# Litianyu141/Gen-FVGN-steady

Measured on AMD Instinct MI355X. Metric: training iters/sec, 50k-cell cylinder mesh (fwd + loss + bwd + Adam, batch resident in HBM), higher is better.
Workload: dtype f32

## Files before the change

### gen-fvgn-steady_amd/csrc/cfwd.hip

```cpp
#include <cstdlib>

#include "tchain_kernel.h"

#include "gfv_limits.h"
int* gfv_internal_status_ptr();

namespace {

constexpr float CF_SH = 16.0f;
constexpr float CF_SH_INV = 1.0f / 16.0f;
constexpr float CF_SH_LIMIT = 2048.0f;

__device__ __forceinline__ void cf_barrier() {
  asm volatile("s_waitcnt lgkmcnt(0)\n\ts_barrier" ::: "memory");
}

template <int KT0, int TG, int NW>
struct CfLds {
  static constexpr int KTB = KT0 > 4 ? KT0 : 4;
  static constexpr int B0 = 0;
  static constexpr int B1 = TG * KTB * 2048;
  static constexpr int SINV = B1 + TG * 8192;
  static constexpr int LNP = SINV + TG * 64;
  static constexpr int TOTAL = LNP + TG * 16 * NW * 8;
};

template <int KT0, int N0, int TG, bool PADD, int LOWP, bool RAGIN, int NW = 4, bool FINLN = true>
__global__ __launch_bounds__(64 * NW, NW == 8 ? 4 : 2) void cfwd_kernel(const gfv_rowtile_args_t A, int* status) {
  static_assert(TG == 2 || TG == 4, "one loader wave per group");
  static_assert(NW == 4 || NW == 8, "32 or 16 columns per wave");
  constexpr int NT = 8 / NW;
  using LY = CfLds<KT0, TG, NW>;
  constexpr bool BF = LOWP == 2;
  __shared__ __attribute__((aligned(16))) char lds[LY::TOTAL];
  char* b0 = lds + LY::B0;
  char* b1 = lds + LY::B1;
  float* sinv = reinterpret_cast<float*>(lds + LY::SINV);
  float* lnp = reinterpret_cast<float*>(lds + LY::LNP);

  const int w = __builtin_amdgcn_readfirstlane(threadIdx.x >> 6);
  const int lane = threadIdx.x & 63, j = lane & 15, g = lane >> 4;
  const int tile = PADD ? gfv_xcd_tile(blockIdx.x, gridDim.x) : (int)blockIdx.x;
  const int row0 = tile * (16 * TG);
  if (row0 >= A.M) return;
  const int ngt = min(TG, (A.M - row0 + 15) >> 4);
  const int c0 = 16 * NT * w + 4 * g;
  const float invw = 1.0f / gfv_pow2_scale(*A.wmax);

  gfv_f16x8 wh[NT][KT0 > 4 ? KT0 : 4], wl[NT][KT0 > 4 ? KT0 : 4];
  {
    const gfv_f16x8* im = reinterpret_cast<const gfv_f16x8*>(A.layer[0].Wh) + (size_t)(NT * w) * 128 + lane;
#pragma unroll
    for (int T = 0; T < KT0; ++T)
#pragma unroll
      for (int n = 0; n < NT; ++n) {
        wh[n][T] = im[T * 1024 + n * 128];
        if (!LOWP) wl[n][T] = im[T * 1024 + n * 128 + 64];
      }
  }
  float4 ps[PADD ? TG : 1][NT], pr[PADD ? TG : 1][NT];
  if (PADD) {
#pragma unroll
    for (int q = 0; q < TG; ++q) {
      const int row = min(row0 + 16 * q + j, A.M - 1);
      const float* s = A.padd + (size_t)A.padd_s[row] * A.padd_ld + c0;
      const float* r = A.padd + (size_t)A.padd_r[row] * A.padd_ld + 128 + c0;
#pragma unroll
      for (int n = 0; n < NT; ++n) { ps[q][n] = ld4(s + 16 * n); pr[q][n] = ld4(r + 16 * n); }
    }
  }
  if (w < TG) {
    const int row = min(row0 + 16 * w + j, A.M - 1);
    float v[2 * KT0][4];
    if (RAGIN) {
      const int width = A.seg[0].width;
      const float* rp = A.seg[0].ptr + (size_t)row * A.seg[0].ld;
#pragma unroll
      for (int u = 0; u < 2; ++u)
#pragma unroll
        for (int e = 0; e < 4; ++e) {
          const int col = 16 * u + 4 * g + e;
          v[u][e] = col < width ? rp[col] : 0.f;
        }
    } else {
      const float* p0 = A.seg[0].ptr + (size_t)row * A.seg[0].ld + 4 * g;
      const float* p1 = p0;
      if (N0 < 2 * KT0) p1 = A.seg[1].ptr + (size_t)row * A.seg[1].ld + 4 * g;
#pragma unroll
      for (int u = 0; u < 2 * KT0; ++u) {
        const float4 t = ld4(u < N0 ? p0 + 16 * u : p1 + 16 * (u - N0));
        v[u][0] = t.x; v[u][1] = t.y; v[u][2] = t.z; v[u][3] = t.w;
      }
    }
    float m0 = 0.f, m1 = 0.f;
#pragma unroll
    for (int u = 0; u < 2 * KT0; ++u) {
      m0 = max3_abs(m0, v[u][0], v[u][1]);
      m1 = max3_abs(m1, v[u][2], v[u][3]);
    }
    const float s = gfv_pow2_scale(row_max4(max3_abs(0.f, m0, m1)));
    if (g == 0) sinv[w * 16 + j] = 1.0f / s;
    gfv_uint4* dst = reinterpret_cast<gfv_uint4*>(b0 + (size_t)w * KT0 * 2048) + lane;
#pragma unroll
    for (int T = 0; T < KT0; ++T) {
      float e[8];
#pragma unroll
      for (int r = 0; r < 4; ++r) { e[r] = v[2 * T][r] * s; e[4 + r] = v[2 * T + 1][r] * s; }
      gfv_uint4 hi, lo;
      gfv_split8_t<BF>(e, hi, lo);
      dst[(2 * T) * 64] = hi;
      if (!LOWP) dst[(2 * T + 1) * 64] = lo;
    }
  }
  float4 bias[3][NT];
#pragma unroll
  for (int l = 0; l < 3; ++l) {
    const float* bp = (FINLN || l < 2) ? A.layer[l].bias : nullptr;
#pragma unroll
    for (int n = 0; n < NT; ++n) bias[l][n] = bp ? ld4(bp + c0 + 16 * n) : make_float4(0.f, 0.f, 0.f, 0.f);
  }
  float mabs = 0.f;
  cf_barrier();

  floatx4 acc[TG][NT];
  auto mma = [&](const char* xbuf, auto ktc) {
    constexpr int KT = decltype(ktc)::value;
#pragma unroll
    for (int q = 0; q < TG; ++q)
#pragma unroll
      for (int n = 0; n < NT; ++n) acc[q][n] = floatx4{0.f, 0.f, 0.f, 0.f};
#pragma unroll
    for (int T = 0; T < KT; ++T) {
#pragma unroll
      for (int q = 0; q < TG; ++q) {
        const gfv_f16x8* f = reinterpret_cast<const gfv_f16x8*>(xbuf + (size_t)(q * KT + T) * 2048) + lane;
        const gfv_f16x8 xh = f[0];
        if (!LOWP) {
          const gfv_f16x8 xl = f[64];
#pragma unroll
          for (int n = 0; n < NT; ++n) {
            acc[q][n] = __builtin_amdgcn_mfma_f32_16x16x32_f16(wl[n][T], xh, acc[q][n], 0, 0, 0);
            acc[q][n] = __builtin_amdgcn_mfma_f32_16x16x32_f16(wh[n][T], xl, acc[q][n], 0, 0, 0);
          }
        }
#pragma unroll
        for (int n = 0; n < NT; ++n) acc[q][n] = gfv_mma_hh<BF>(wh[n][T], xh, acc[q][n]);
      }
    }
  };
  auto load_w = [&](const void* image) {
    const gfv_f16x8* im = reinterpret_cast<const gfv_f16x8*>(image) + (size_t)(NT * w) * 128 + lane;
#pragma unroll
    for (int T = 0; T < 4; ++T)
#pragma unroll
      for (int n = 0; n < NT; ++n) {
        wh[n][T] = im[T * 1024 + n * 128];
        if (!LOWP) wl[n][T] = im[T * 1024 + n * 128 + 64];
      }
  };
  auto hidden = [&](int layer, char* xout, float* save) {
#pragma unroll
    for (int q = 0; q < TG; ++q) {
      const int row = row0 + 16 * q + j;
      const bool live = q < ngt && row < A.M;
      const float si = layer == 0 ? sinv[q * 16 + j] : CF_SH_INV;
      float a[4 * NT];
#pragma unroll
      for (int n = 0; n < NT; ++n) {
        const float4 b = bias[layer][n];
        float v[4] = {(acc[q][n][0] * si) * invw + b.x, (acc[q][n][1] * si) * invw + b.y, (acc[q][n][2] * si) * invw + b.z,
                      (acc[q][n][3] * si) * invw + b.w};
        if (PADD && layer == 0) {
          v[0] += ps[PADD ? q : 0][n].x + pr[PADD ? q : 0][n].x; v[1] += ps[PADD ? q : 0][n].y + pr[PADD ? q : 0][n].y;
          v[2] += ps[PADD ? q : 0][n].z + pr[PADD ? q : 0][n].z; v[3] += ps[PADD ? q : 0][n].w + pr[PADD ? q : 0][n].w;
        }
        if (save && live) st4(save + (size_t)row * 128 + c0 + 16 * n, v);
        const gfv_f2 g01 = gfv_gelu2(gfv_f2{v[0], v[1]}), g23 = gfv_gelu2(gfv_f2{v[2], v[3]});
        a[4 * n + 0] = g01.x; a[4 * n + 1] = g01.y; a[4 * n + 2] = g23.x; a[4 * n + 3] = g23.y;
      }
      float m = 0.f;
#pragma unroll
      for (int e = 0; e < 4 * NT; e += 2) m = max3_abs(m, a[e], a[e + 1]);
      mabs = fmaxf(mabs, live ? m : 0.f);
      if constexpr (NT == 2) {
        float e8[8];
#pragma unroll
        for (int e = 0; e < 8; ++e) e8[e] = a[e] * CF_SH;
        gfv_uint4 hi, lo;
        gfv_split8_t<BF>(e8, hi, lo);
        gfv_uint4* dst = reinterpret_cast<gfv_uint4*>(xout + (size_t)(q * 4 + w) * 2048) + lane;
        dst[0] = hi;
        if (!LOWP) dst[64] = lo;
      } else {
        unsigned h0, h1, l0, l1;
        gfv_split_pair_t<BF>(a[0] * CF_SH, a[1] * CF_SH, h0, l0);
        gfv_split_pair_t<BF>(a[2] * CF_SH, a[3] * CF_SH, h1, l1);
        char* dst = xout + (size_t)(q * 4 + (w >> 1)) * 2048 + lane * 16 + (w & 1) * 8;
        *reinterpret_cast<uint2*>(dst) = make_uint2(h0, h1);
        if (!LOWP) *reinterpret_cast<uint2*>(dst + 1024) = make_uint2(l0, l1);
      }
    }
  };

  mma(b0, std::integral_constant<int, KT0>{});
  load_w(A.layer[1].Wh);
  hidden(0, b1, A.layer[0].save);
  cf_barrier();
  mma(b1, std::integral_constant<int, 4>{});
  load_w(A.layer[2].Wh);
  hidden(1, b0, A.layer[1].save);
  float4 gam[NT], bet[NT];
  if constexpr (FINLN) {
#pragma unroll
    for (int n = 0; n < NT; ++n) { gam[n] = ld4(A.fin_gamma + c0 + 16 * n); bet[n] = ld4(A.fin_beta + c0 + 16 * n); }
  }
  float4 rres[TG][NT];
  if (A.res[0]) {
#pragma unroll
    for (int q = 0; q < TG; ++q) {
      const float* rp = A.res[0] + (size_t)min(row0 + 16 * q + j, A.M - 1) * A.res_ld[0] + c0;
#pragma unroll
      for (int n = 0; n < NT; ++n) rres[q][n] = ld4(rp + 16 * n);
    }
  }
  cf_barrier();
  if constexpr (!FINLN) {
    if (w == 0) {
      mma(b0, std::integral_constant<int, 4>{});
      const int ncol = A.layer[2].N;
      const float* bp = A.layer[2].bias;
#pragma unroll
      for (int q = 0; q < TG; ++q) {
        const int row = row0 + 16 * q + j;
        if (q < ngt && row < A.M) {
#pragma unroll
          for (int r = 0; r < 4; ++r) {
            const int col = 4 * g + r;
            if (col < ncol) A.out[0][(size_t)row * A.out_ld[0] + col] = (acc[q][0][r] * CF_SH_INV) * invw + (bp ? bp[col] : 0.f);
          }
        }
      }
    }
    if (mabs > CF_SH_LIMIT) atomicOr(status, 2);
    return;
  }
  mma(b0, std::integral_constant<int, 4>{});
  const int hcols = (A.hidden > 0 && A.hidden < 128) ? A.hidden : 128;
  float y[TG][4 * NT];
#pragma unroll
  for (int q = 0; q < TG; ++q) {
    const int row = row0 + 16 * q + j;
    const bool live = q < ngt && row < A.M;
    float s = 0.f;
#pragma unroll
    for (int n = 0; n < NT; ++n) {
      const float4 b = bias[2][n];
      float v[4] = {(acc[q][n][0] * CF_SH_INV) * invw + b.x, (acc[q][n][1] * CF_SH_INV) * invw + b.y,
                    (acc[q][n][2] * CF_SH_INV) * invw + b.z, (acc[q][n][3] * CF_SH_INV) * invw + b.w};
      if (A.fin_presave && live) st4(A.fin_presave + (size_t)row * 128 + c0 + 16 * n, v);
#pragma unroll
      for (int r = 0; r < 4; ++r) {
        y[q][4 * n + r] = v[r];
        s += v[r];
      }
    }
    const float mw = row_sum(s) * (1.0f / (16.0f * NT));
    float m2 = 0.f;
#pragma unroll
    for (int e = 0; e < 4 * NT; ++e) {
      const float d = y[q][e] - mw;
      m2 += d * d;
    }
    m2 = row_sum(m2);
    if (g == 0) *reinterpret_cast<float2*>(lnp + ((q * 16 + j) * NW + w) * 2) = make_float2(mw, m2);
  }
  cf_barrier();
  {
    const float inv_h = 1.0f / (float)hcols, npad = (float)(128 - hcols);
#pragma unroll
    for (int q = 0; q < TG; ++q) {
      const int row = row0 + 16 * q + j;
      const bool live = q < ngt && row < A.M;
      const float4* pp = reinterpret_cast<const float4*>(lnp + (q * 16 + j) * 2 * NW);
      float m128, m2a;
      if constexpr (NW == 4) {
        const float4 p0 = pp[0], p1 = pp[1];
        m128 = ((p0.x + p0.z) + (p1.x + p1.z)) * 0.25f;
        const float e0 = p0.x - m128, e1 = p0.z - m128, e2 = p1.x - m128, e3 = p1.z - m128;
        m2a = ((p0.y + p0.w) + (p1.y + p1.w)) + 32.0f * ((e0 * e0 + e1 * e1) + (e2 * e2 + e3 * e3));
      } else {
        const float4 p0 = pp[0], p1 = pp[1], p2 = pp[2], p3 = pp[3];
        m128 = (((p0.x + p0.z) + (p1.x + p1.z)) + ((p2.x + p2.z) + (p3.x + p3.z))) * 0.125f;
        const float e0 = p0.x - m128, e1 = p0.z - m128, e2 = p1.x - m128, e3 = p1.z - m128, e4 = p2.x - m128, e5 = p2.z - m128,
                    e6 = p3.x - m128, e7 = p3.z - m128;
        m2a = (((p0.y + p0.w) + (p1.y + p1.w)) + ((p2.y + p2.w) + (p3.y + p3.w))) +
              16.0f * (((e0 * e0 + e1 * e1) + (e2 * e2 + e3 * e3)) + ((e4 * e4 + e5 * e5) + (e6 * e6 + e7 * e7)));
      }
      const float mean = hcols == 128 ? m128 : (m128 * 128.0f) * inv_h;
      const float dm = m128 - mean;
      const float m2 = hcols == 128 ? m2a : (m2a + 128.0f * dm * dm) - npad * (mean * mean);
      const float rstd = rsqrtf(m2 * inv_h + 1e-5f);
      if (A.fin_stats && live && w == 0 && g == 0) *reinterpret_cast<float2*>(A.fin_stats + 2 * (size_t)row) = make_float2(mean, rstd);
#pragma unroll
      for (int n = 0; n < NT; ++n) {
        const float4 ga = gam[n], be = bet[n];
        float o[4] = {(y[q][4 * n + 0] - mean) * rstd * ga.x + be.x, (y[q][4 * n + 1] - mean) * rstd * ga.y + be.y,
                      (y[q][4 * n + 2] - mean) * rstd * ga.z + be.z, (y[q][4 * n + 3] - mean) * rstd * ga.w + be.w};
        if (live) {
          if (A.out_nores) st4(A.out_nores + (size_t)row * 128 + c0 + 16 * n, o);
          if (A.res[0]) { o[0] += rres[q][n].x; o[1] += rres[q][n].y; o[2] += rres[q][n].z; o[3] += rres[q][n].w; }
          st4(A.out[0] + (size_t)row * A.out_ld[0] + c0 + 16 * n, o);
        }
      }
    }
  }
  if (mabs > CF_SH_LIMIT) atomicOr(status, 2);
}

inline bool cf_al16(const void* p) { return (reinterpret_cast<size_t>(p) & 15) == 0; }

template <int KT0, int N0, bool PADD, bool RAGIN, bool FINLN = true>
void cf_launch(const gfv_rowtile_args_t& a, int lowp, hipStream_t stream) {
  int* st = gfv_internal_status_ptr();
  constexpr int tg = 2;
  const int tiles = (a.M + 16 * tg - 1) / (16 * tg);
  const dim3 grid(PADD ? gfv_xcd_grid(tiles) : tiles), blk(512);
  if (lowp == 2) GFV_LAUNCH((cfwd_kernel<KT0, N0, 2, PADD, 2, RAGIN, 8, FINLN>), grid, blk, 0, stream, a, st);
  else if (lowp) GFV_LAUNCH((cfwd_kernel<KT0, N0, 2, PADD, 1, RAGIN, 8, FINLN>), grid, blk, 0, stream, a, st);
  else GFV_LAUNCH((cfwd_kernel<KT0, N0, 2, PADD, 0, RAGIN, 8, FINLN>), grid, blk, 0, stream, a, st);
}

}

int gfv_internal_cfwd_try(const gfv_rowtile_args_t* a, int lowp, hipStream_t stream, int dry) {
  if (!gfv_internal_status_ptr()) return 0;
  const int on = gfv_internal_limit(GFV_LIM_CFWD_ON);
  const int max_m = gfv_internal_limit(GFV_LIM_CFWD_MAX_M);
  if (!on || a->nlayers != 3 || a->M > max_m || a->M < 1 || (a->flags & (GFV_CHAIN_ROW_OWNER | GFV_CHAIN_COLUMN_OWNER))) return 0;
  const bool dec = a->fin_op == GFV_FIN_PLAIN && a->layer[2].N >= 1 && a->layer[2].N <= 16 && !a->res[0] && !a->out_nores && !a->fin_presave &&
                   !a->fin_stats && !a->padd && a->nseg == 1 && a->layer[0].K == 128;
  if (a->in_op != GFV_IN_NONE || !a->wmax) return 0;
  if (!dec && (a->fin_op != GFV_FIN_LN || !a->fin_gamma || !a->fin_beta)) return 0;
  if (a->in_add || a->gadd || a->in_save || a->in_aux || a->ln_partial || a->gscale || a->dw_partial || a->in_stats || a->fin_aux) return 0;
  for (int l = 0; l < 3; ++l) {
    const gfv_layer_t& L = a->layer[l];
    if (!L.Wh || (L.N != 128 && !(dec && l == 2)) || L.aux || L.bias2 || (L.bias && !cf_al16(L.bias) && !(dec && l == 2))) return 0;
    if (L.op != (l < 2 ? GFV_OP_BIAS_GELU : GFV_OP_NONE)) return 0;
    if (l > 0 && L.K != 128) return 0;
    if (L.save && !cf_al16(L.save)) return 0;
  }
  if (a->layer[2].save) return 0;
  if (!a->out[0] || a->out[1] || a->out[2] || (!dec && ((a->out_ld[0] & 3) || !cf_al16(a->out[0]))) || a->res[1] || a->res[2]) return 0;
  if (a->res[0] && ((a->res_ld[0] & 3) || !cf_al16(a->res[0]))) return 0;
  if ((a->out_nores && !cf_al16(a->out_nores)) || (a->fin_presave && !cf_al16(a->fin_presave)) ||
      (!dec && (!cf_al16(a->fin_gamma) || !cf_al16(a->fin_beta))))
    return 0;
  if (a->fin_stats && (reinterpret_cast<size_t>(a->fin_stats) & 7)) return 0;
  for (int i = 0; i < a->nseg; ++i)
    if (a->seg[i].idx || a->seg[i].csr_rowptr || a->seg[i].csr_scale || a->seg[i].save) return 0;
  const int K0 = a->layer[0].K;
  int shape = -1;
  auto plain = [&](int i, int width) {
    const gfv_seg_t& s = a->seg[i];
    return s.width == width && (s.ld & 3) == 0 && cf_al16(s.ptr);
  };
  if (a->padd) {
    if (a->nseg == 1 && K0 == 128 && plain(0, 128) && a->padd_s && a->padd_r && a->padd_ld >= 256 && (a->padd_ld & 3) == 0 && cf_al16(a->padd))
      shape = 1;
  } else if (a->nseg == 2 && K0 == 192 && plain(0, 64) && plain(1, 128)) {
    shape = 0;
  } else if (dec) {
    if (plain(0, 128)) shape = 4;
  } else if (a->nseg == 1 && K0 == 128 && plain(0, 128)) {
    shape = 2;
  } else if (a->nseg == 1 && K0 <= 32 && a->seg[0].width == K0) {
    shape = 3;
  }
  if (shape < 0) return 0;
  if (dry) return 1;
  if (shape == 0) cf_launch<6, 4, false, false>(*a, lowp, stream);
  else if (shape == 1) cf_launch<4, 8, true, false>(*a, lowp, stream);
  else if (shape == 2) cf_launch<4, 8, false, false>(*a, lowp, stream);
  else if (shape == 4) cf_launch<4, 8, false, false, false>(*a, lowp, stream);
  else cf_launch<1, 2, false, true>(*a, lowp, stream);
  return 1;
}
```

### gen-fvgn-steady_amd/csrc/gfv_limits.h

```cpp
#pragma once
enum {
  GFV_LIM_CBWD_ON = 0,
  GFV_LIM_CBWD_MAX_M,
  GFV_LIM_CFWD_ON,
  GFV_LIM_CFWD_MAX_M,
  GFV_LIM_CTRANS_ON,
  GFV_LIM_CTRANS_MAX_M,
  GFV_LIM_LIN1S_ON,
  GFV_LIM_LIN1S_MAX_M,
  GFV_LIM_COUNT
};
int gfv_internal_limit(int which);
```

### gen-fvgn-steady_amd/csrc/rowtile.hip

```cpp
#include <atomic>
#include <stdio.h>
#include <stdlib.h>
#include <mutex>
#include "gfv_common.h"
#include "gfv_limits.h"
#include "gfv_prof.h"
#include "../../include/gfv.h"

namespace {
constexpr int BM = 64;
}

int gfv_internal_tchain_launch(const gfv_rowtile_args_t* args, int ragged, int f16, hipStream_t stream);

static std::atomic<int> g_f16_default{-1};
static thread_local int g_f16split = -1;
static int f16_default() {
  int d = g_f16_default.load(std::memory_order_relaxed);
  if (d < 0) {
    const char* e = getenv("GFV_F16SPLIT");
    d = e ? ((atoi(e) == 2 || atoi(e) == 3) ? atoi(e) : (atoi(e) != 0)) : 1;
    int expect = -1;
    if (!g_f16_default.compare_exchange_strong(expect, d)) d = expect;
  }
  return d;
}
extern "C" int gfv_f16split_enabled(void) { return g_f16split >= 0 ? g_f16split : f16_default(); }
extern "C" int gfv_set_f16split(int32_t on) {
  g_f16_default.store((on == 2 || on == 3) ? on : (on ? 1 : 0));
  g_f16split = -1;
  return GFV_OK;
}
extern "C" int gfv_set_f16split_thread(int32_t on) {
  if (on < -1 || on > 3) return GFV_ERR_ARG;
  g_f16split = on;
  return GFV_OK;
}
static int f16_mode() { return gfv_f16split_enabled(); }

static thread_local int g_hidden = 128;
extern "C" int gfv_hidden_size(void) { return g_hidden; }
extern "C" int gfv_set_hidden_size(int32_t h) {
  if (h < 16 || h > 128 || (h & 15)) return GFV_ERR_ARG;
  g_hidden = h;
  return GFV_OK;
}

static thread_local int g_last_path = -1;
extern "C" int gfv_rowtile_last_path(void) { return g_last_path; }
namespace {
struct LimitDef { const char* env; int dflt; };
const LimitDef k_limits[GFV_LIM_COUNT] = {
    {"GFV_CBWD", 1},        {"GFV_CBWD_MAX_M", 25000},      {"GFV_CFWD", 1},          {"GFV_CFWD_MAX_M", 250000},
    {"GFV_CTRANS", 1},         {"GFV_CTRANS_MAX_M", 16384},
    {"GFV_LIN1S", 1},       {"GFV_LIN1S_MAX_M", 16384}};
int g_limit[GFV_LIM_COUNT];
bool g_limit_set[GFV_LIM_COUNT];
std::once_flag g_limit_once;
void limits_init() {
  for (int i = 0; i < GFV_LIM_COUNT; ++i) {
    const char* e = getenv(k_limits[i].env);
    g_limit[i] = e ? atoi(e) : k_limits[i].dflt;
    g_limit_set[i] = false;
  }
}
}
int gfv_internal_limit(int which) {
  std::call_once(g_limit_once, limits_init);
  return (which >= 0 && which < GFV_LIM_COUNT) ? g_limit[which] : 0;
}
extern "C" int gfv_get_limit(int32_t which) { return (which >= 0 && which < GFV_LIM_COUNT) ? gfv_internal_limit(which) : -1; }
extern "C" int gfv_set_limit(int32_t which, int32_t value) {
  if (which < 0 || which >= GFV_LIM_COUNT) return GFV_ERR_ARG;
  std::call_once(g_limit_once, limits_init);
  if (value < 0) {
    const char* e = getenv(k_limits[which].env);
    g_limit[which] = e ? atoi(e) : k_limits[which].dflt;
  } else {
    g_limit[which] = value;
  }
  return GFV_OK;
}
extern "C" const char* gfv_limit_name(int32_t which) { return (which >= 0 && which < GFV_LIM_COUNT) ? k_limits[which].env : nullptr; }

static thread_local int g_last_ln_rows = 0;
extern "C" int gfv_rowtile_last_ln_rows(void) { return g_last_ln_rows; }

extern "C" int gfv_rowtile_tiles(int32_t M) { return (M + BM - 1) / BM; }

static int rowtile_chain_impl(const gfv_rowtile_args_t* args, void* stream);
extern "C" int gfv_rowtile_chain(const gfv_rowtile_args_t* args, void* stream) {
  if (!args) return GFV_ERR_ARG;
  if (args->product_form < 0 || args->product_form > 4 || (args->hidden != 0 && (args->hidden < 16 || args->hidden > 128 || (args->hidden & 15))))
    return GFV_ERR_ARG;
  if (args->product_form == 0 && args->hidden == 0) return rowtile_chain_impl(args, stream);
  const int f0 = g_f16split, h0 = g_hidden;
  if (args->product_form) g_f16split = args->product_form - 1;
  if (args->hidden) g_hidden = args->hidden;
  const int rc = rowtile_chain_impl(args, stream);
  g_f16split = f0;
  g_hidden = h0;
  return rc;
}
int gfv_internal_lin1_try(const gfv_rowtile_args_t* a, int lowp, hipStream_t stream, int dry);
int gfv_internal_cfwd_try(const gfv_rowtile_args_t* a, int lowp, hipStream_t stream, int dry);
bool gfv_internal_wimg_form_ok(const float* wmax);
int gfv_internal_cbwd_try(const gfv_rowtile_args_t* a, int lowp, hipStream_t stream, int dry);
static int cfwd_try(const gfv_rowtile_args_t* args, int lowp, hipStream_t stream, int dry) {
  if (args->nlayers != 3 || (args->fin_op != GFV_FIN_LN && args->fin_op != GFV_FIN_PLAIN)) return 0;
  gfv_rowtile_args_t local = *args;
  local.hidden = g_hidden;
  return gfv_internal_cfwd_try(&local, lowp, stream, dry);
}
static int cbwd_try(const gfv_rowtile_args_t* args, int lowp, hipStream_t stream, int dry) {
  if (args->in_op != GFV_IN_LNBWD || args->dw_partial || !args->in_stats) return 0;
  gfv_rowtile_args_t local = *args;
  local.hidden = g_hidden;
  return gfv_internal_cbwd_try(&local, lowp, stream, dry);
}
static int rowtile_chain_impl(const gfv_rowtile_args_t* args, void* stream) {
  if (!args || args->M < 0 || args->nlayers < 1 || args->nlayers > 3 || args->nseg < 1 || args->nseg > 3) return GFV_ERR_ARG;
  if (args->M == 0) {
    g_last_ln_rows = 0;
    return GFV_OK;
  }
  for (int i = 0; i < args->nseg; ++i)
    if (args->seg[i].width < 1 || args->seg[i].width > 128) return GFV_ERR_ARG;
  for (int l = 0; l + 1 < args->nlayers; ++l)
    if (args->layer[l].N != 128 || args->layer[l + 1].K != 128) return GFV_ERR_ARG;
  int k0 = 0;
  for (int i = 0; i < args->nseg; ++i) k0 += args->seg[i].width;
  if (k0 != args->layer[0].K) return GFV_ERR_ARG;
  const gfv_layer_t& last = args->layer[args->nlayers - 1];
  if (last.N > 384 || last.N < 1) return GFV_ERR_ARG;
  if ((args->rc_Wh[0] || args->rc_Wh[1]) && !args->dw_partial) return GFV_ERR_ARG;
  if (args->padd && (args->nlayers < 2 || args->padd_ld < 256 || (args->padd_ld & 3) || !args->padd_s || !args->padd_r)) return GFV_ERR_ARG;
  for (int l = 0; l < args->nlayers; ++l)
    if (args->layer[l].ldw != 0 && args->layer[l].ldw < args->layer[l].K) return GFV_ERR_ARG;
  if (last.N > 128 && (last.N & 15)) return GFV_ERR_ARG;
  if ((args->fin_op != GFV_FIN_PLAIN || args->in_op == GFV_IN_LN || args->in_op == GFV_IN_LNBWD) &&
      (args->fin_op != GFV_FIN_PLAIN ? last.N != 128 : false))
    return GFV_ERR_ARG;
  if ((args->in_op == GFV_IN_LN || args->in_op == GFV_IN_LNBWD) && (args->nseg != 1 || args->seg[0].width != 128))
    return GFV_ERR_ARG;
  bool fast_t = true;
  for (int i = 0; i < args->nseg; ++i) fast_t = fast_t && (args->seg[i].width % 32 == 0) && (args->seg[i].ld % 4 == 0);
  for (int l = 0; l < args->nlayers; ++l) {
    const bool lastl = (l == args->nlayers - 1);
    fast_t = fast_t && (args->layer[l].K % 4 == 0) && (args->layer[l].ldw % 4 == 0) && (args->layer[l].N % (lastl ? 64 : 128) == 0);
  }
  if (args->fin_op != GFV_FIN_PLAIN) fast_t = fast_t && last.N == 128;
  for (int c = 0; c < 3; ++c) {
    if (args->out[c]) fast_t = fast_t && (args->out_ld[c] % 4 == 0);
    if (args->res[c]) fast_t = fast_t && (args->res_ld[c] % 4 == 0);
  }
  bool rag_t = !fast_t && args->in_op != GFV_IN_LNBWD && args->fin_op != GFV_FIN_LNBWD;
  for (int l = 0; l + 1 < args->nlayers; ++l) rag_t = rag_t && args->layer[l].N == 128;
  if (last.N > 128) rag_t = rag_t && (last.N % 64 == 0);
  if (last.N % 16) rag_t = rag_t && last.op != GFV_OP_MUL_DGELU && args->fin_op == GFV_FIN_PLAIN && !args->out_nores;
  if (args->in_op == GFV_IN_LN) rag_t = rag_t && args->seg[0].width == 128 && (args->seg[0].ld % 4 == 0);
  if (args->gadd) rag_t = rag_t && args->seg[0].width == 128 && (args->seg[0].ld % 4 == 0);
  for (int l = 1; l < args->nlayers; ++l) rag_t = rag_t && (args->layer[l].K == 128);
  {
    bool csr = false;
    for (int i = 0; i < args->nseg; ++i) {
      const gfv_seg_t& sg = args->seg[i];
      csr = csr || sg.csr_rowptr != nullptr || sg.save != nullptr;
      if (sg.csr_rowptr && (!sg.idx || (i == 0 && args->in_add))) return GFV_ERR_ARG;
    }
    if (csr && (!fast_t || args->in_op == GFV_IN_LNBWD || args->fin_op == GFV_FIN_LNBWD))
      return GFV_ERR_ARG;
  }
  bool f16 = (fast_t || rag_t) && f16_mode() != 0 && args->wmax != nullptr;
  for (int l = 0; l < args->nlayers; ++l) f16 = f16 && args->layer[l].Wh != nullptr;
  for (int i = 0; i + 1 < args->nseg; ++i) f16 = f16 && (args->seg[i].width % 32 == 0);
  if (f16 && !gfv_internal_wimg_form_ok(args->wmax)) return GFV_ERR_ARG;
  for (int l = 0; l < args->nlayers; ++l)
    if ((!args->layer[l].W || args->layer[l].bias2) && !f16) return GFV_ERR_ARG;
  if (!fast_t && !rag_t) {
    static const bool dbg = getenv("GFV_ROWTILE_DEBUG") != nullptr;
    if (dbg)
      fprintf(stderr, "[gfv] gfv_rowtile_chain: unsupported shape M=%d nseg=%d widths=%d,%d,%d ld0=%d nlayers=%d K0=%d Nlast=%d out_ld=%d in_op=%d fin_op=%d\n",
              args->M, args->nseg, args->seg[0].width, args->nseg > 1 ? args->seg[1].width : 0,
              args->nseg > 2 ? args->seg[2].width : 0, args->seg[0].ld, args->nlayers, args->layer[0].K, last.N,
              args->out_ld[0], args->in_op, args->fin_op);
    return GFV_ERR_ARG;
  }
  void* tok = nullptr;
  if (gfv_prof_enabled()) {
    double fl = 0, by = 0;
    for (int l = 0; l < args->nlayers; ++l) {
      fl += 2.0 * args->M * (double)args->layer[l].K * args->layer[l].N;
      by += 4.0 * ((double)args->layer[l].K * args->layer[l].N + args->layer[l].N);
      if (args->layer[l].save) by += 4.0 * args->M * args->layer[l].N;
      if (args->layer[l].aux) by += 4.0 * args->M * args->layer[l].N;
    }
    by += 4.0 * args->M * (double)args->layer[0].K + 4.0 * args->M * (double)last.N;
    for (int i = 0; i < args->nseg; ++i) if (args->seg[i].idx) by += 4.0 * args->M;
    if (args->in_aux || args->fin_aux) by += 4.0 * args->M * 128.0;
    if (args->in_save) by += 4.0 * args->M * 128.0;
    if (args->fin_presave) by += 4.0 * args->M * 128.0;
    if (args->out_nores) by += 4.0 * args->M * 128.0;
    if (args->padd) by += 4.0 * args->M * 258.0;
    for (int c = 0; c < 3; ++c) if (args->res[c]) by += 4.0 * args->M * 128.0;
    const int lnm = args->in_op == GFV_IN_LNBWD ? 1 : (args->fin_op == GFV_FIN_LNBWD ? 2 : 0);
    int kind = fast_t ? GFV_K_TCHAIN0 + lnm : GFV_K_TCHAIN_RAG;
    for (int i = 0; i < args->nseg; ++i)
      if (args->seg[i].csr_rowptr || args->seg[i].save) kind = GFV_K_TCHAIN_CSR;
    if (fast_t && f16 && args->nlayers == 1 && gfv_internal_lin1_try(args, f16_mode() >= 2 ? f16_mode() - 1 : 0, (hipStream_t)stream, 1))
      kind = GFV_K_LIN1;
    if (f16 && cfwd_try(args, f16_mode() >= 2 ? f16_mode() - 1 : 0, (hipStream_t)stream, 1))
      kind = GFV_K_COLCHAIN_FWD;
    if (args->dw_partial) {
      kind = GFV_K_COLCHAIN_BWD;
      const int nfused = 2 + (args->rc_Wh[0] ? 2 : 0);
      fl += nfused * 2.0 * args->M * 128.0 * 128.0;
      by += 8.0 * args->M + 4.0 * (double)gfv_rowtile_dw_partials_m(args->M) * (double)args->dw_partial_stride;
    }
    tok = gfv_prof_begin(kind, fl, by, (hipStream_t)stream);
  }
  g_last_path = (fast_t ? 1 : 2) + (f16 ? 4 : 0);
  g_last_ln_rows = (args->M + BM - 1) / BM;
  if (args->dw_partial && !(fast_t && f16)) return GFV_ERR_ARG;
  if (fast_t && f16 && args->nlayers == 1 && gfv_internal_lin1_try(args, f16_mode() >= 2 ? f16_mode() - 1 : 0, (hipStream_t)stream, 0)) {
    g_last_path += 32;
  } else if (f16 && !args->dw_partial && cfwd_try(args, f16_mode() >= 2 ? f16_mode() - 1 : 0, (hipStream_t)stream, 0)) {
    g_last_path += 64;
  } else if (fast_t && f16 && cbwd_try(args, f16_mode() >= 2 ? f16_mode() - 1 : 0, (hipStream_t)stream, 0)) {
    g_last_path += 128;
    g_last_ln_rows = (args->M + 31) / 32;
  } else if (fast_t) {
    const int took = gfv_internal_tchain_launch(args, 0, f16 ? 1 : 0, (hipStream_t)stream);
    if (args->dw_partial && took != 2) return GFV_ERR_ARG;
    g_last_path += 8 * took;
  }
  else
    gfv_internal_tchain_launch(args, 1, f16 ? 1 : 0, (hipStream_t)stream);
  gfv_prof_end(tok, (hipStream_t)stream);
  GFV_CHECK_LAUNCH();
  return GFV_OK;
}
```

Measured before the change: 285.4.

## Raise cfwd occupancy target by cutting register pressure and streaming next-layer weights

The fused forward MLP kernel now takes a min-waves launch-bound parameter that defaults to 6 waves per SIMD instead of 4, selectable through a new GFV_CFWD_MIN_WAVES limit. To fit that register budget it splits the first-layer weight registers, keeps only two bias sets live, and defers the gather of the sender and receiver addends until after staging. It also loads the next layer's weights one k-step at a time inside the MFMA loop behind scheduling barriers, and rematerialises lane-derived indices to shorten live ranges. LDS is padded to 56KB at the lower occupancy setting. The risk is spills or exposed load latency at the higher occupancy target, since this kernel is only one part of the training step.

```diff
diff --git a/gen-fvgn-steady_amd/csrc/cfwd.hip b/gen-fvgn-steady_amd/csrc/cfwd.hip
--- a/gen-fvgn-steady_amd/csrc/cfwd.hip
+++ b/gen-fvgn-steady_amd/csrc/cfwd.hip
@@ -25,51 +25,65 @@
   static constexpr int TOTAL = LNP + TG * 16 * NW * 8;
 };
 
-template <int KT0, int N0, int TG, bool PADD, int LOWP, bool RAGIN, int NW = 4, bool FINLN = true>
-__global__ __launch_bounds__(64 * NW, NW == 8 ? 4 : 2) void cfwd_kernel(const gfv_rowtile_args_t A, int* status) {
+constexpr int CF_LDS_TWO = 56 * 1024;
+template <int V>
+using cf_ic = std::integral_constant<int, V>;
+
+template <int KT0, int N0, int TG, bool PADD, int LOWP, bool RAGIN, int NW, bool FINLN, int MINW>
+__global__ __launch_bounds__(64 * NW, MINW) void cfwd_kernel(const gfv_rowtile_args_t A, int* status) {
   static_assert(TG == 2 || TG == 4, "one loader wave per group");
   static_assert(NW == 4 || NW == 8, "32 or 16 columns per wave");
   constexpr int NT = 8 / NW;
+  constexpr int KH = KT0 > 4 ? 2 : KT0;
+  constexpr int KR = KT0 - KH;
   using LY = CfLds<KT0, TG, NW>;
   constexpr bool BF = LOWP == 2;
-  __shared__ __attribute__((aligned(16))) char lds[LY::TOTAL];
+  __shared__ __attribute__((aligned(16))) char lds[MINW >= 6 || LY::TOTAL > CF_LDS_TWO ? LY::TOTAL : CF_LDS_TWO];
   char* b0 = lds + LY::B0;
   char* b1 = lds + LY::B1;
   float* sinv = reinterpret_cast<float*>(lds + LY::SINV);
   float* lnp = reinterpret_cast<float*>(lds + LY::LNP);
 
   const int w = __builtin_amdgcn_readfirstlane(threadIdx.x >> 6);
-  const int lane = threadIdx.x & 63, j = lane & 15, g = lane >> 4;
+  int lane = threadIdx.x & 63, j = lane & 15, g = lane >> 4;
   const int tile = PADD ? gfv_xcd_tile(blockIdx.x, gridDim.x) : (int)blockIdx.x;
   const int row0 = tile * (16 * TG);
   if (row0 >= A.M) return;
   const int ngt = min(TG, (A.M - row0 + 15) >> 4);
-  const int c0 = 16 * NT * w + 4 * g;
+  int c0 = 16 * NT * w + 4 * g;
+  auto phase = [&]() {
+    asm volatile("" : "+v"(lane));
+    j = lane & 15;
+    g = lane >> 4;
+    c0 = 16 * NT * w + 4 * g;
+  };
   const float invw = 1.0f / gfv_pow2_scale(*A.wmax);
 
-  gfv_f16x8 wh[NT][KT0 > 4 ? KT0 : 4], wl[NT][KT0 > 4 ? KT0 : 4];
-  {
-    const gfv_f16x8* im = reinterpret_cast<const gfv_f16x8*>(A.layer[0].Wh) + (size_t)(NT * w) * 128 + lane;
-#pragma unroll
-    for (int T = 0; T < KT0; ++T)
+  auto load_w = [&](const void* image, auto& h, auto& l, int T0, int F, int KT) {
+    const gfv_f16x8* im = reinterpret_cast<const gfv_f16x8*>(image) + (size_t)(NT * w) * 128 + lane;
+#pragma unroll
+    for (int T = F; T < F + KT; ++T)
 #pragma unroll
       for (int n = 0; n < NT; ++n) {
-        wh[n][T] = im[T * 1024 + n * 128];
-        if (!LOWP) wl[n][T] = im[T * 1024 + n * 128 + 64];
-      }
-  }
-  float4 ps[PADD ? TG : 1][NT], pr[PADD ? TG : 1][NT];
+        h[n][T] = im[(T0 + T) * 1024 + n * 128];
+        if (!LOWP) l[n][T] = im[(T0 + T) * 1024 + n * 128 + 64];
+      }
+  };
+  gfv_f16x8 wh[NT][4], wl[NT][4];
+  gfv_f16x8 wh2[NT][KR ? KR : 1], wl2[NT][KR ? KR : 1];
+  load_w(A.layer[0].Wh, wh, wl, 0, 0, KH);
+  int is[PADD ? TG : 1], ir[PADD ? TG : 1];
   if (PADD) {
 #pragma unroll
     for (int q = 0; q < TG; ++q) {
       const int row = min(row0 + 16 * q + j, A.M - 1);
-      const float* s = A.padd + (size_t)A.padd_s[row] * A.padd_ld + c0;
-      const float* r = A.padd + (size_t)A.padd_r[row] * A.padd_ld + 128 + c0;
-#pragma unroll
-      for (int n = 0; n < NT; ++n) { ps[q][n] = ld4(s + 16 * n); pr[q][n] = ld4(r + 16 * n); }
-    }
-  }
-  if (w < TG) {
+      is[q] = A.padd_s[row];
+      ir[q] = A.padd_r[row];
+    }
+  }
+  if (w >= TG) {
+    if constexpr (KR > 0) load_w(A.layer[0].Wh, wh2, wl2, KH, 0, KR);
+  } else {
     const int row = min(row0 + 16 * w + j, A.M - 1);
     float v[2 * KT0][4];
     if (RAGIN) {
@@ -110,55 +124,65 @@
       gfv_split8_t<BF>(e, hi, lo);
       dst[(2 * T) * 64] = hi;
       if (!LOWP) dst[(2 * T + 1) * 64] = lo;
-    }
-  }
-  float4 bias[3][NT];
-#pragma unroll
-  for (int l = 0; l < 3; ++l) {
+      if (T < KR) load_w(A.layer[0].Wh, wh2, wl2, KH, T, 1);
+    }
+  }
+  float4 ps[PADD ? TG : 1][NT], pr[PADD ? TG : 1][NT];
+  if (PADD) {
+#pragma unroll
+    for (int q = 0; q < TG; ++q) {
+      const float* s = A.padd + (size_t)is[q] * A.padd_ld + c0;
+      const float* r = A.padd + (size_t)ir[q] * A.padd_ld + 128 + c0;
+#pragma unroll
+      for (int n = 0; n < NT; ++n) { ps[q][n] = ld4(s + 16 * n); pr[q][n] = ld4(r + 16 * n); }
+    }
+  }
+  float4 bias[2][NT];
+  auto load_bias = [&](int l) {
     const float* bp = (FINLN || l < 2) ? A.layer[l].bias : nullptr;
 #pragma unroll
-    for (int n = 0; n < NT; ++n) bias[l][n] = bp ? ld4(bp + c0 + 16 * n) : make_float4(0.f, 0.f, 0.f, 0.f);
-  }
+    for (int n = 0; n < NT; ++n) bias[l & 1][n] = bp ? ld4(bp + c0 + 16 * n) : make_float4(0.f, 0.f, 0.f, 0.f);
+  };
+  load_bias(0);
   float mabs = 0.f;
   cf_barrier();
 
   floatx4 acc[TG][NT];
-  auto mma = [&](const char* xbuf, auto ktc) {
-    constexpr int KT = decltype(ktc)::value;
-#pragma unroll
-    for (int q = 0; q < TG; ++q)
-#pragma unroll
-      for (int n = 0; n < NT; ++n) acc[q][n] = floatx4{0.f, 0.f, 0.f, 0.f};
-#pragma unroll
-    for (int T = 0; T < KT; ++T) {
+  auto mma = [&](const char* xbuf, const auto& h, const auto& l, auto ktc, auto t0c, auto kpc, const void* next) {
+    constexpr int KT = decltype(ktc)::value, T0 = decltype(t0c)::value, KP = decltype(kpc)::value;
+    if constexpr (T0 == 0) {
+#pragma unroll
+      for (int q = 0; q < TG; ++q)
+#pragma unroll
+        for (int n = 0; n < NT; ++n) acc[q][n] = floatx4{0.f, 0.f, 0.f, 0.f};
+    }
+#pragma unroll
+    for (int T = 0; T < KP; ++T) {
 #pragma unroll
       for (int q = 0; q < TG; ++q) {
-        const gfv_f16x8* f = reinterpret_cast<const gfv_f16x8*>(xbuf + (size_t)(q * KT + T) * 2048) + lane;
+        const gfv_f16x8* f = reinterpret_cast<const gfv_f16x8*>(xbuf + (size_t)(q * KT + T0 + T) * 2048) + lane;
         const gfv_f16x8 xh = f[0];
         if (!LOWP) {
           const gfv_f16x8 xl = f[64];
 #pragma unroll
           for (int n = 0; n < NT; ++n) {
-            acc[q][n] = __builtin_amdgcn_mfma_f32_16x16x32_f16(wl[n][T], xh, acc[q][n], 0, 0, 0);
-            acc[q][n] = __builtin_amdgcn_mfma_f32_16x16x32_f16(wh[n][T], xl, acc[q][n], 0, 0, 0);
+            acc[q][n] = __builtin_amdgcn_mfma_f32_16x16x32_f16(l[n][T], xh, acc[q][n], 0, 0, 0);
+            acc[q][n] = __builtin_amdgcn_mfma_f32_16x16x32_f16(h[n][T], xl, acc[q][n], 0, 0, 0);
           }
         }
 #pragma unroll
-        for (int n = 0; n < NT; ++n) acc[q][n] = gfv_mma_hh<BF>(wh[n][T], xh, acc[q][n]);
-      }
-    }
-  };
-  auto load_w = [&](const void* image) {
-    const gfv_f16x8* im = reinterpret_cast<const gfv_f16x8*>(image) + (size_t)(NT * w) * 128 + lane;
-#pragma unroll
-    for (int T = 0; T < 4; ++T)
-#pragma unroll
-      for (int n = 0; n < NT; ++n) {
-        wh[n][T] = im[T * 1024 + n * 128];
-        if (!LOWP) wl[n][T] = im[T * 1024 + n * 128 + 64];
-      }
-  };
+        for (int n = 0; n < NT; ++n) acc[q][n] = gfv_mma_hh<BF>(h[n][T], xh, acc[q][n]);
+      }
+      if (next) {
+        if (T < 4) load_w(next, wh, wl, 0, T, 1);
+        __builtin_amdgcn_sched_barrier(0x78f);
+      }
+    }
+    if (next && KP < 4) load_w(next, wh, wl, 0, KP, 4 - KP);
+  };
+  auto mma128 = [&](const char* xbuf, const void* next) { mma(xbuf, wh, wl, cf_ic<4>{}, cf_ic<0>{}, cf_ic<4>{}, next); };
   auto hidden = [&](int layer, char* xout, float* save) {
+    phase();
 #pragma unroll
     for (int q = 0; q < TG; ++q) {
       const int row = row0 + 16 * q + j;
@@ -167,7 +191,7 @@
       float a[4 * NT];
 #pragma unroll
       for (int n = 0; n < NT; ++n) {
-        const float4 b = bias[layer][n];
+        const float4 b = bias[layer & 1][n];
         float v[4] = {(acc[q][n][0] * si) * invw + b.x, (acc[q][n][1] * si) * invw + b.y, (acc[q][n][2] * si) * invw + b.z,
                       (acc[q][n][3] * si) * invw + b.w};
         if (PADD && layer == 0) {
@@ -182,6 +206,7 @@
 #pragma unroll
       for (int e = 0; e < 4 * NT; e += 2) m = max3_abs(m, a[e], a[e + 1]);
       mabs = fmaxf(mabs, live ? m : 0.f);
+      asm volatile("" : "+v"(mabs));
       if constexpr (NT == 2) {
         float e8[8];
 #pragma unroll
@@ -202,13 +227,19 @@
     }
   };
 
-  mma(b0, std::integral_constant<int, KT0>{});
-  load_w(A.layer[1].Wh);
+  if constexpr (KR > 0) {
+    mma(b0, wh, wl, cf_ic<KT0>{}, cf_ic<0>{}, cf_ic<KH>{}, nullptr);
+    mma(b0, wh2, wl2, cf_ic<KT0>{}, cf_ic<KH>{}, cf_ic<KR>{}, A.layer[1].Wh);
+  } else {
+    mma(b0, wh, wl, cf_ic<KT0>{}, cf_ic<0>{}, cf_ic<KH>{}, A.layer[1].Wh);
+  }
+  load_bias(1);
   hidden(0, b1, A.layer[0].save);
   cf_barrier();
-  mma(b1, std::integral_constant<int, 4>{});
-  load_w(A.layer[2].Wh);
+  mma128(b1, A.layer[2].Wh);
+  load_bias(2);
   hidden(1, b0, A.layer[1].save);
+  phase();
   float4 gam[NT], bet[NT];
   if constexpr (FINLN) {
 #pragma unroll
@@ -226,7 +257,7 @@
   cf_barrier();
   if constexpr (!FINLN) {
     if (w == 0) {
-      mma(b0, std::integral_constant<int, 4>{});
+      mma128(b0, nullptr);
       const int ncol = A.layer[2].N;
       const float* bp = A.layer[2].bias;
 #pragma unroll
@@ -244,7 +275,8 @@
     if (mabs > CF_SH_LIMIT) atomicOr(status, 2);
     return;
   }
-  mma(b0, std::integral_constant<int, 4>{});
+  mma128(b0, nullptr);
+  phase();
   const int hcols = (A.hidden > 0 && A.hidden < 128) ? A.hidden : 128;
   float y[TG][4 * NT];
 #pragma unroll
@@ -254,7 +286,7 @@
     float s = 0.f;
 #pragma unroll
     for (int n = 0; n < NT; ++n) {
-      const float4 b = bias[2][n];
+      const float4 b = bias[0][n];
       float v[4] = {(acc[q][n][0] * CF_SH_INV) * invw + b.x, (acc[q][n][1] * CF_SH_INV) * invw + b.y,
                     (acc[q][n][2] * CF_SH_INV) * invw + b.z, (acc[q][n][3] * CF_SH_INV) * invw + b.w};
       if (A.fin_presave && live) st4(A.fin_presave + (size_t)row * 128 + c0 + 16 * n, v);
@@ -275,6 +307,7 @@
     if (g == 0) *reinterpret_cast<float2*>(lnp + ((q * 16 + j) * NW + w) * 2) = make_float2(mw, m2);
   }
   cf_barrier();
+  phase();
   {
     const float inv_h = 1.0f / (float)hcols, npad = (float)(128 - hcols);
 #pragma unroll
@@ -319,15 +352,21 @@
 
 inline bool cf_al16(const void* p) { return (reinterpret_cast<size_t>(p) & 15) == 0; }
 
-template <int KT0, int N0, bool PADD, bool RAGIN, bool FINLN = true>
-void cf_launch(const gfv_rowtile_args_t& a, int lowp, hipStream_t stream) {
+template <int KT0, int N0, bool PADD, bool RAGIN, bool FINLN, int MINW>
+void cf_launch_w(const gfv_rowtile_args_t& a, int lowp, hipStream_t stream) {
   int* st = gfv_internal_status_ptr();
   constexpr int tg = 2;
   const int tiles = (a.M + 16 * tg - 1) / (16 * tg);
   const dim3 grid(PADD ? gfv_xcd_grid(tiles) : tiles), blk(512);
-  if (lowp == 2) GFV_LAUNCH((cfwd_kernel<KT0, N0, 2, PADD, 2, RAGIN, 8, FINLN>), grid, blk, 0, stream, a, st);
-  else if (lowp) GFV_LAUNCH((cfwd_kernel<KT0, N0, 2, PADD, 1, RAGIN, 8, FINLN>), grid, blk, 0, stream, a, st);
-  else GFV_LAUNCH((cfwd_kernel<KT0, N0, 2, PADD, 0, RAGIN, 8, FINLN>), grid, blk, 0, stream, a, st);
+  if (lowp == 2) GFV_LAUNCH((cfwd_kernel<KT0, N0, 2, PADD, 2, RAGIN, 8, FINLN, MINW>), grid, blk, 0, stream, a, st);
+  else if (lowp) GFV_LAUNCH((cfwd_kernel<KT0, N0, 2, PADD, 1, RAGIN, 8, FINLN, MINW>), grid, blk, 0, stream, a, st);
+  else GFV_LAUNCH((cfwd_kernel<KT0, N0, 2, PADD, 0, RAGIN, 8, FINLN, MINW>), grid, blk, 0, stream, a, st);
+}
+
+template <int KT0, int N0, bool PADD, bool RAGIN, bool FINLN = true, bool THREE = true>
+void cf_launch(const gfv_rowtile_args_t& a, int lowp, hipStream_t stream) {
+  if (!THREE || gfv_internal_limit(GFV_LIM_CFWD_MIN_WAVES) == 4) cf_launch_w<KT0, N0, PADD, RAGIN, FINLN, 4>(a, lowp, stream);
+  else if constexpr (THREE) cf_launch_w<KT0, N0, PADD, RAGIN, FINLN, 6>(a, lowp, stream);
 }
 
 }
@@ -378,7 +417,7 @@
   }
   if (shape < 0) return 0;
   if (dry) return 1;
-  if (shape == 0) cf_launch<6, 4, false, false>(*a, lowp, stream);
+  if (shape == 0) cf_launch<6, 4, false, false, true, false>(*a, lowp, stream);
   else if (shape == 1) cf_launch<4, 8, true, false>(*a, lowp, stream);
   else if (shape == 2) cf_launch<4, 8, false, false>(*a, lowp, stream);
   else if (shape == 4) cf_launch<4, 8, false, false, false>(*a, lowp, stream);
diff --git a/gen-fvgn-steady_amd/csrc/gfv_limits.h b/gen-fvgn-steady_amd/csrc/gfv_limits.h
--- a/gen-fvgn-steady_amd/csrc/gfv_limits.h
+++ b/gen-fvgn-steady_amd/csrc/gfv_limits.h
@@ -8,6 +8,7 @@
   GFV_LIM_CTRANS_MAX_M,
   GFV_LIM_LIN1S_ON,
   GFV_LIM_LIN1S_MAX_M,
+  GFV_LIM_CFWD_MIN_WAVES,
   GFV_LIM_COUNT
 };
 int gfv_internal_limit(int which);
diff --git a/gen-fvgn-steady_amd/csrc/rowtile.hip b/gen-fvgn-steady_amd/csrc/rowtile.hip
--- a/gen-fvgn-steady_amd/csrc/rowtile.hip
+++ b/gen-fvgn-steady_amd/csrc/rowtile.hip
@@ -53,7 +53,7 @@
 const LimitDef k_limits[GFV_LIM_COUNT] = {
     {"GFV_CBWD", 1},        {"GFV_CBWD_MAX_M", 25000},      {"GFV_CFWD", 1},          {"GFV_CFWD_MAX_M", 250000},
     {"GFV_CTRANS", 1},         {"GFV_CTRANS_MAX_M", 16384},
-    {"GFV_LIN1S", 1},       {"GFV_LIN1S_MAX_M", 16384}};
+    {"GFV_LIN1S", 1},       {"GFV_LIN1S_MAX_M", 16384},     {"GFV_CFWD_MIN_WAVES", 6}};
 int g_limit[GFV_LIM_COUNT];
 bool g_limit_set[GFV_LIM_COUNT];
 std::once_flag g_limit_once;
```

New measurement: 284.6. No clear change (-0.3%).
